# febrianrachmadi/dep-gan-im

Measured on AMD Instinct MI355X. Metric: 2D slices/sec (G+2D+GP train step), 256x256x1 fp32, higher is better.
Workload: dtype f32; 1 GPU; DEP-GAN-IM twoCritics canonical train step (critic-Y2 + critic-DEM + G update, WGAN-GP), batch 32 per GPU, 256x256x1; per_gpu_batch=32, global_batch=32, parallelism=dp1

## Files before the change

dep_gan_im_amd/csrc/common.h:

```cpp
#pragma once
#include <hip/hip_runtime.h>
#include <stdint.h>
#include <stddef.h>

typedef float f32x2 __attribute__((ext_vector_type(2)));
typedef float f32x4 __attribute__((ext_vector_type(4)));
typedef float f32x16 __attribute__((ext_vector_type(16)));

struct TView {
  float* p;
  long sB, sY, sX;
};

static inline TView make_view(float* p, int H, int W, int C) {
  TView v;
  v.p = p;
  v.sX = C;
  v.sY = (long)W * C;
  v.sB = (long)H * W * C;
  return v;
}
static inline TView make_view_slice(float* p, int H, int W, int Ctot, int c0) {
  TView v = make_view(p, H, W, Ctot);
  v.p = p + c0;
// ... 217 lines not shown
int dg_wino_epi_class(unsigned flags, int form);
void dg_set_epi_classes(int on);
int dg_get_epi_classes();
void dg_conv_igemm_name(const ConvPlan& pl, const ConvArgs& a, char* buf, size_t cap);
int dg_conv_direct(int KS, const ConvArgs& a, hipStream_t st);

size_t dg_wgrad_part_floats(int KS, int B, int H, int W, int Cin, int Cout);
int dg_wgrad(int KS, const WgradArgs& a, int* nchunks, hipStream_t st);
int dg_wgrad_finish(const float* part, int nchunks, int ntaps, int Cin, int Cout, const float* scale, float* out,
                    float* raw, int accumulate, int oi, const float* colpart, int colC, const float* colscale,
                    float* colout, float* colraw, hipStream_t st);
int dg_wgrad_finish_rows(const float* part, int nchunks, int ntaps, int Cin, int Cout, const float* scale, float* out,
                         float* raw, int accumulate, int oi, const float* colpart, int colrows, int colC,
                         const float* colscale, float* colout, float* colraw, hipStream_t st);
int dg_wgrad_reduce(const float* part, int nchunks, int ntaps, int Cin, int Cout, const float* scale, float* out,
                    float* raw, int accumulate, int oi, hipStream_t st);

bool dg_wgrad_bf16_supported(int KS, int Cin, int Cout);
size_t dg_wgrad_bf16_part_floats(int KS, int B, int H, int W, int Cin, int Cout);
int dg_wgrad_bf16(int KS, const WgradArgs& a, int* nchunks, hipStream_t st);

size_t dg_wgrad_small_part_floats(int KS, int B, int H, int W, int Cin, int Cout);
int dg_wgrad_small(int KS, const WgradArgs& a, int* nchunks, hipStream_t st);

int dg_wgrad_plan(int KS, int B, int H, int W, int Cin, int Cout, int out[4]);
int dg_wgrad_small_plan(int KS, int B, int H, int W, int Cin, int Cout, int out[4]);
int dg_wgrad_bf16_plan(int KS, int B, int H, int W, int Cin, int Cout, int out[4]);
```

dep_gan_im_amd/csrc/direct.hip:

```cpp
#include "common.h"
#include "epilogue.h"

template <int KS, int COG, int G>
__global__ __launch_bounds__(256) void conv_direct_kernel(const ConvArgs a) {
  constexpr int PAD = KS / 2;
  constexpr int TW = 16 + KS - 1;
  constexpr int PIXT = TW * TW;
  constexpr int NTAPS = KS * KS;
  constexpr int CT = COG * G;
  constexpr int CIK = 8;
  constexpr int PPP = 256 / G;
  constexpr int NPASS = G;

  extern __shared__ __attribute__((aligned(16))) float smem[];
  float* xs = smem;
  float* ws = smem + CIK * PIXT;

  const int tid = threadIdx.x;
  const int tilesX = (a.W + 15) >> 4, tilesY = (a.H + 15) >> 4;
  int t = blockIdx.x;
  const int tx0 = (t % tilesX) * 16;
  t /= tilesX;
  const int ty0 = (t % tilesY) * 16;
  const int b = t / tilesY;
// ... 349 lines not shown
      const int iy = ty0 + (pix >> 4), ix = tx0 + (pix & 15);
      float v = 0.f;
      if (iy < a.H && ix < a.W) v = a.dy.p[view_off(a.dy, b, iy, ix) + c];
      ds[pix * a.Cout + c] = v;
    }
    __syncthreads();
    for (int py = 0; py < 16; ++py)
#pragma unroll 4
      for (int px = 0; px < 16; ++px) {
        const int xo = py * TW + px;
        const int dof = (py * 16 + px) * a.Cout;
#pragma unroll
        for (int k = 0; k < NOUT; ++k) acc[k] = fmaf(xs[xoff[k] + xo], ds[dof + co_[k]], acc[k]);
      }
  }
  float* pout = a.part + (size_t)blockIdx.x * nout;
#pragma unroll
  for (int k = 0; k < NOUT; ++k) {
    const int o = tid + k * 256;
    if (o < nout) pout[o] = acc[k];
  }
}

template <int KS>
__global__ __launch_bounds__(256) void wgrad_edge_kernel(const WgradArgs a) {
  constexpr int PAD = KS / 2;
  constexpr int TW = 16 + KS - 1;
  constexpr int PIXT = TW * TW;
  constexpr int NTAPS = KS * KS;
  extern __shared__ __attribute__((aligned(16))) float smem[];
  const int xsz = (a.Cin * PIXT + 3) & ~3;
  float* xs = smem;
  float* ds = smem + xsz;
  const int tid = threadIdx.x, lane = tid & 63, wv = tid >> 6;
  const int i = lane & 15, kq = lane >> 4;
  const int M = NTAPS * a.Cin;
  const int MT = (M + 15) >> 4, NTl = a.Cout >> 4;
  int aoff[2];
  bool aval[2];
#pragma unroll
  for (int mt = 0; mt < 2; ++mt) {
    const int m = mt * 16 + i;
    aval[mt] = m < M;
    const int mm = aval[mt] ? m : 0;
    const int tap = mm / a.Cin, ci = mm - tap * a.Cin;
    aoff[mt] = ci * PIXT + (tap / KS) * TW + (tap % KS);
  }
  f32x4 acc[2][2];
#pragma unroll
  for (int mt = 0; mt < 2; ++mt)
#pragma unroll
    for (int nt = 0; nt < 2; ++nt) acc[mt][nt] = (f32x4){0.f, 0.f, 0.f, 0.f};
  const int tilesX = (a.W + 15) >> 4, tilesY = (a.H + 15) >> 4;
  const int t0 = blockIdx.x * a.tilesPerChunk, t1 = min(t0 + a.tilesPerChunk, a.nTiles);
  const int C4 = a.Cout >> 2;
  for (int tile = t0; tile < t1; ++tile) {
    int t = tile;
    const int tx0 = (t % tilesX) * 16;
    t /= tilesX;
    const int ty0 = (t % tilesY) * 16;
    const int b = t / tilesY;
    __syncthreads();
    for (int q = tid; q < PIXT * a.Cin; q += 256) {
      const int pix = q / a.Cin, c = q - pix * a.Cin;
      const int ly = pix / TW, lx = pix - ly * TW;
      const int iy = ty0 + ly - PAD, ix = tx0 + lx - PAD;
      float v = 0.f;
      if (iy >= 0 && iy < a.H && ix >= 0 && ix < a.W) v = a.x.p[view_off(a.x, b, iy, ix) + c];
      xs[c * PIXT + pix] = v;
    }
    for (int q = tid; q < 256 * C4; q += 256) {
      const int pix = q / C4, c = (q - pix * C4) * 4;
      const int iy = ty0 + (pix >> 4), ix = tx0 + (pix & 15);
      f32x4 v = {0.f, 0.f, 0.f, 0.f};
      if (iy < a.H && ix < a.W) v = *reinterpret_cast<const f32x4*>(a.dy.p + view_off(a.dy, b, iy, ix) + c);
      *reinterpret_cast<f32x4*>(ds + pix * a.Cout + c) = v;
    }
    __syncthreads();
#pragma unroll 4
    for (int kk = 0; kk < 16; ++kk) {
      const int kl = kk * 4 + kq;
      const int py = 4 * wv + (kl >> 4), px = kl & 15;
      const int po = py * TW + px;
      float av[2], bv[2];
#pragma unroll
      for (int mt = 0; mt < 2; ++mt) av[mt] = aval[mt] ? xs[aoff[mt] + po] : 0.f;
#pragma unroll
      for (int nt = 0; nt < 2; ++nt) bv[nt] = (nt < NTl) ? ds[(py * 16 + px) * a.Cout + nt * 16 + i] : 0.f;
#pragma unroll
      for (int mt = 0; mt < 2; ++mt)
#pragma unroll
        for (int nt = 0; nt < 2; ++nt)
          if (mt < MT && nt < NTl) acc[mt][nt] = __builtin_amdgcn_mfma_f32_16x16x4f32(av[mt], bv[nt], acc[mt][nt], 0, 0, 0);
    }
  }
  __syncthreads();
  float* red = smem;
#pragma unroll
  for (int mt = 0; mt < 2; ++mt)
#pragma unroll
    for (int nt = 0; nt < 2; ++nt)
#pragma unroll
      for (int j = 0; j < 4; ++j) red[wv * 1024 + (mt * 16 + 4 * kq + j) * 32 + nt * 16 + i] = acc[mt][nt][j];
  __syncthreads();
  float* pout = a.part + (size_t)blockIdx.x * M * a.Cout;
  for (int e = tid; e < M * a.Cout; e += 256) {
    const int m = e / a.Cout, n = e - m * a.Cout;
    const int o = m * 32 + n;
    pout[e] = (red[o] + red[1024 + o]) + (red[2048 + o] + red[3072 + o]);
  }
}

static void small_chunking(int B, int H, int W, int* nTiles, int* tpc, int* nch) {
  *nTiles = B * cdiv(W, 16) * cdiv(H, 16);
  int want = *nTiles / 6;
  if (want < 1024) want = 1024;
  if (want > 8192) want = 8192;
  if (want > *nTiles) want = *nTiles;
  *tpc = cdiv(*nTiles, want);
  *nch = cdiv(*nTiles, *tpc);
}

size_t dg_wgrad_small_part_floats(int KS, int B, int H, int W, int Cin, int Cout) {
  int nTiles, tpc, nch;
  small_chunking(B, H, W, &nTiles, &tpc, &nch);
  const size_t slab = (size_t)KS * KS * Cin * Cout;
  return (size_t)nch * slab;
}

int dg_wgrad_small_plan(int KS, int B, int H, int W, int Cin, int Cout, int out[4]) {
  if (KS * KS * Cin * Cout > 1024 || Cout > 64) {
    dg_set_error("dg_wgrad_small: taps*Cin*Cout = %d too large", KS * KS * Cin * Cout);
    return DG_ERR_UNSUPPORTED;
  }
  if (KS != 3 && KS != 5) {
    dg_set_error("dg_wgrad_small: unsupported kernel size %d", KS);
    return DG_ERR_UNSUPPORTED;
  }
  small_chunking(B, H, W, &out[0], &out[1], &out[2]);
  out[3] = 1;
  return DG_OK;
}

int dg_wgrad_small(int KS, const WgradArgs& a_in, int* nchunks, hipStream_t st) {
  WgradArgs a = a_in;
  if (KS * KS * a.Cin * a.Cout > 1024 || a.Cout > 64) {
    dg_set_error("dg_wgrad_small: taps*Cin*Cout = %d too large", KS * KS * a.Cin * a.Cout);
    return DG_ERR_UNSUPPORTED;
  }
  int nTiles, tpc, nch;
  small_chunking(a.B, a.H, a.W, &nTiles, &tpc, &nch);
  a.nTiles = nTiles;
  a.tilesPerChunk = tpc;
  *nchunks = nch;
  const int TW = 16 + KS - 1;
  const bool edge = (KS * KS * a.Cin <= 32) && (a.Cout == 16 || a.Cout == 32) && (a.dy.sX % 4 == 0) &&
                    (a.dy.sY % 4 == 0) && (a.dy.sB % 4 == 0);
  if (edge) {
    size_t lds = (size_t)(((a.Cin * TW * TW + 3) & ~3) + 256 * a.Cout) * sizeof(float);
    if (lds < 4 * 1024 * sizeof(float)) lds = 4 * 1024 * sizeof(float);
    if (KS == 3)
      hipLaunchKernelGGL(wgrad_edge_kernel<3>, dim3(nch), dim3(256), lds, st, a);
    else if (KS == 5)
      hipLaunchKernelGGL(wgrad_edge_kernel<5>, dim3(nch), dim3(256), lds, st, a);
    else {
      dg_set_error("dg_wgrad_small: unsupported kernel size %d", KS);
      return DG_ERR_UNSUPPORTED;
    }
    HIPCHECK(hipGetLastError());
    return DG_OK;
  }
  const size_t lds = (size_t)(a.Cin * TW * TW + 256 * a.Cout) * sizeof(float);
  if (KS == 3)
    hipLaunchKernelGGL(wgrad_small_kernel<3>, dim3(nch), dim3(256), lds, st, a);
  else if (KS == 5)
    hipLaunchKernelGGL(wgrad_small_kernel<5>, dim3(nch), dim3(256), lds, st, a);
  else {
    dg_set_error("dg_wgrad_small: unsupported kernel size %d", KS);
    return DG_ERR_UNSUPPORTED;
  }
// ... 4 lines not shown
```

dep_gan_im_amd/csrc/model.hip:

```cpp
#include "model.h"
#include "train_ops.h"

#include <dlfcn.h>
#include <float.h>
#include <math.h>
#include <stdlib.h>
#include <stdarg.h>
#include <stdio.h>
#include <string.h>

static thread_local char g_err[1024] = "";
void dg_set_error(const char* fmt, ...) {
  va_list ap;
  va_start(ap, fmt);
  vsnprintf(g_err, sizeof(g_err), fmt, ap);
  va_end(ap);
}
const char* dg_get_error() { return g_err; }

void Net::add(const std::string& name, std::vector<int> shape, bool trainable) {
  PInfo pi;
  pi.name = name;
  pi.ndim = (int)shape.size();
  pi.size = 1;
// ... 198 lines not shown
  int nch = 0;
  const double fl = 2.0 * N * H * W * (double)Cin * Cout * KS * KS;
  char lb[56];
  snprintf(lb, sizeof(lb), "wgrad k%d b%d %dx%d %d->%d", KS, N, H, W, Cin, Cout);
  const bool mfma = Cin % 4 == 0 && Cout % 4 == 0 && Cin >= 8;
  if (ws.bf16 && mfma && dg_wgrad_bf16_supported(KS, Cin, Cout)) {
    if (dg_wgrad_bf16_part_floats(KS, N, H, W, Cin, Cout) > ws.partFloats) {
      dg_set_error("wgrad slab workspace too small");
      return DG_ERR_ARG;
    }
    if (cs) {
      a.colpart = scratch;
      a.colB = cs->B;
    }
    snprintf(lb, sizeof(lb), "wgrad(bf16) k%d b%d %dx%d %d->%d", KS, N, H, W, Cin, Cout);
    {
      ProfScope ps(c, 1, fl, lb);
      DGCHECK(dg_wgrad_bf16(KS, a, &nch, ws.st));
    }
    ProfScope ps(c, 2, 0.0, "slab reduce");
    return dg_wgrad_finish(ws.part, nch, KS * KS, Cin, Cout, scale, out, raw, accumulate, oi, cs ? scratch : nullptr,
                           Cout, cs ? cs->scale : nullptr, cs ? cs->out : nullptr, cs ? cs->raw : nullptr, ws.st);
  }
  if (cs && !mfma) {
    ProfScope ps(c, 2, 0.0, "colsum");
    DGCHECK(dg_colsum(dy, cs->B, H, W, Cout, cs->scale, cs->out, cs->raw, 0, scratch, cap, ws.st));
  }
  if (mfma) {
    if (dg_wgrad_part_floats(KS, N, H, W, Cin, Cout) > ws.partFloats) {
      dg_set_error("wgrad slab workspace too small");
      return DG_ERR_ARG;
    }
    if (cs) {
      a.colpart = scratch;
      a.colB = cs->B;
    }
    {
      ProfScope ps(c, 1, fl, lb);
      DGCHECK(dg_wgrad(KS, a, &nch, ws.st));
    }
    ProfScope ps(c, 2, 0.0, "slab reduce");
    return dg_wgrad_finish(ws.part, nch, KS * KS, Cin, Cout, scale, out, raw, accumulate, oi, cs ? scratch : nullptr,
                           Cout, cs ? cs->scale : nullptr, cs ? cs->out : nullptr, cs ? cs->raw : nullptr, ws.st);
  } else {
    if (dg_wgrad_small_part_floats(KS, N, H, W, Cin, Cout) > ws.partFloats) {
      dg_set_error("wgrad slab workspace too small");
      return DG_ERR_ARG;
    }
    ProfScope ps(c, 2, fl, lb);
    DGCHECK(dg_wgrad_small(KS, a, &nch, ws.st));
  }
  ProfScope ps(c, 2, 0.0, "slab reduce");
  return dg_wgrad_reduce(ws.part, nch, KS * KS, Cin, Cout, scale, out, raw, accumulate, oi, ws.st);
}
int wgrad_full(depgan_ctx* c, int KS, TView x, TView dy, int N, int H, int W, int Cin, int Cout,
               const float* scale, float* out, float* raw, int accumulate, int oi, const ColSum* cs) {
  const WgradWs ws = {c->part, c->partFloats, c->scratch, c->scratchFloats, c->cfg.bf16_mfma && c->wgrad_bf16, c->st, c};
  return wgrad_run(ws, KS, x, dy, N, H, W, Cin, Cout, scale, out, raw, accumulate, oi, cs);
}

static const char* kHeadSfx[NOISE_NHEADS] = {"add_m3", "mul_m3", "add_m2", "mul_m2", "add_m1", "mul_m1", "add",
                                             "mul",    "add_p3", "mul_p3", "add_p2", "mul_p2", "add_p1", "mul_p1"};
static const int kHeadMult[NOISE_NHEADS] = {3, 3, 2, 2, 1, 1, 4, 4, 3, 3, 2, 2, 1, 1};

struct TrunkEnt {
  GKind kind;
  const char* name;
  int ci, co;
  const char* aux;
};
static const TrunkEnt kTrunk[] = {
    {G_CONV, "gen_0", -1, 1, ""},        {G_FILM, "gen_noise_m1", 1, 1, "m1"}, {G_CONV, "gen_1", 1, 1, ""},
    {G_POOL, "skip1", 0, 0, ""},         {G_CONV, "gen_2", 1, 2, ""},          {G_FILM, "gen_noise_m2", 2, 2, "m2"},
// ... 1507 lines not shown
```

dep_gan_im_amd/csrc/op_entries.hip:

```cpp
#include "model.h"
#include "train_ops.h"

#include <math.h>
#include <stdlib.h>
#include <stdio.h>
#include <string.h>

int op_pack_jobs(PackJob* jobs, int n, hipStream_t st) {
  const unsigned nb = dg_pack_layout(jobs, n);
  DevTmp jd(st);
  DGCHECK(jd.alloc(n * sizeof(PackJob)));
  hipError_t e = hipMemcpyAsync(jd.p, jobs, n * sizeof(PackJob), hipMemcpyHostToDevice, st);
  if (e != hipSuccess) { dg_set_error("op_pack_jobs: upload failed: %s", hipGetErrorString(e)); return DG_ERR_HIP; }
  return dg_pack_weights_batch(jd.as<PackJob>(), n, nb, st);
}

extern "C" {

static int op_conv_run(ConvArgs a, const float* w_hwio, int Cin, int Cout, int KS, int path, int bwd, hipStream_t st) {
  const int ci = a.Cin, co = a.Cout;
  ConvPlan pl = (path == 3) ? dg_plan_conv_bf16(KS, ci, co)
                : (path == 4 || path == 5) ? dg_plan_conv_split(KS, ci, co, path == 5 ? 3 : 2)
                : (path == 6) ? dg_plan_conv_items(KS, ci, co, 1L << 30) : dg_plan_conv(KS, ci, co);
  if (path == 7) pl = dg_plan_conv_items(KS, ci, co, 1L << 30);
// ... 359 lines not shown
                              long dsX, const float* scale, float* dw, float* raw, int accumulate, int oi,
                              int colB, const float* colscale, float* colout, float* colraw, int B, int H, int W,
                              int Cin, int Cout, int KS, int bf16, void* stream) {
  if (op_view_bad_batched(x, xsB, xsY, xsX) || op_view_bad_batched(dy, dsB, dsY, dsX) || !dw || B < 1 || H < 1 || W < 1 || Cin < 1 || Cout < 1 ||
      (KS != 1 && KS != 3 && KS != 5)) {
    dg_set_error("op_conv2d_wgrad_ex: null or non-positive argument");
    return DG_ERR_ARG;
  }
  const bool cols = colout || colraw;
  if ((bf16 != 0 && bf16 != 1) || (cols ? (colB < 1 || colB > B) : (colB != 0 || colscale != nullptr))) {
    dg_set_error("op_conv2d_wgrad_ex: bf16 must be 0 or 1; column sums need colout or colraw and 1 <= colB <= B");
    return DG_ERR_ARG;
  }
  const bool mfma = Cin % 4 == 0 && Cout % 4 == 0 && Cin >= 8;
  if (bf16 && !(mfma && dg_wgrad_bf16_supported(KS, Cin, Cout))) {
    dg_set_error("op_conv2d_wgrad_ex: the bf16 weight-gradient kernel does not cover %d -> %d", Cin, Cout);
    return DG_ERR_UNSUPPORTED;
  }
  hipStream_t st = (hipStream_t)stream;
  WgradWs ws;
  memset(&ws, 0, sizeof(ws));
  ws.partFloats = bf16 ? dg_wgrad_bf16_part_floats(KS, B, H, W, Cin, Cout)
                  : mfma ? dg_wgrad_part_floats(KS, B, H, W, Cin, Cout) : dg_wgrad_small_part_floats(KS, B, H, W, Cin, Cout);
  ws.scratchFloats = mfma ? ws.partFloats / ((size_t)KS * KS * Cin) : (cols ? dg_colsum_scratch(colB, H, W, Cout) : 0);
  ws.bf16 = bf16 != 0;
  ws.st = st;
  DevTmp part(st), scratch(st);
  DGCHECK(op_alloc(&part, ws.partFloats, "op_conv2d_wgrad_ex"));
  DGCHECK(op_alloc(&scratch, ws.scratchFloats, "op_conv2d_wgrad_ex"));
  ws.part = part.as<float>();
  ws.scratch = scratch.as<float>();
  const ColSum cs = {colB, colscale, colout, colraw};
  return wgrad_run(ws, KS, op_view(x, xsB, xsY, xsX), op_view(dy, dsB, dsY, dsX), B, H, W, Cin, Cout, scale, dw, raw, accumulate,
                   oi, cols ? &cs : nullptr);
}

int depgan_debug_wgrad_plan(int kernel, int KS, int B, int H, int W, int Cin, int Cout, int out[4]) {
  if (!out || B < 1 || H < 1 || W < 1 || Cin < 1 || Cout < 1) {
    dg_set_error("debug_wgrad_plan: null or non-positive argument");
    return DG_ERR_ARG;
  }
  switch (kernel) {
    case 0: return dg_wgrad_plan(KS, B, H, W, Cin, Cout, out);
    case 1: return dg_wgrad_small_plan(KS, B, H, W, Cin, Cout, out);
    case 2: return dg_wgrad_bf16_plan(KS, B, H, W, Cin, Cout, out);
    case 3: return dg_wgrad_bf16s_plan(KS, B, H, W, Cin, Cout, out);
    case 4: return dg_deconv_wgrad_plan(B, H, W, Cin, Cout, out);
// ... 584 lines not shown
```

dep_gan_im_amd/csrc/wgrad.hip:

```cpp
#include <stdlib.h>

#include "common.h"

template <int MF>
struct MfmaW;
template <>
struct MfmaW<32> {
  typedef f32x16 acc_t;
  static constexpr int NREG = 16;
  static __device__ __forceinline__ acc_t run(float a, float b, acc_t c) {
    return __builtin_amdgcn_mfma_f32_32x32x2f32(a, b, c, 0, 0, 0);
  }
  static __device__ __forceinline__ int row(int j, int h) { return (j & 3) + 8 * (j >> 2) + 4 * h; }
};
template <>
struct MfmaW<16> {
  typedef f32x4 acc_t;
  static constexpr int NREG = 4;
  static __device__ __forceinline__ acc_t run(float a, float b, acc_t c) {
    return __builtin_amdgcn_mfma_f32_16x16x4f32(a, b, c, 0, 0, 0);
  }
  static __device__ __forceinline__ int row(int j, int h) { return 4 * h + j; }
};

template <int MF, int KS, int TPW, int TH>
struct WDmaCfg {
  static constexpr int TW = 16 + KS - 1, THH = TH + KS - 1, PIXT = THH * TW, V = MF / 4;
  static constexpr int XTOT = PIXT * V, DTOT = TH * 16 * V;
  static constexpr int NXP = (XTOT + 255) / 256, NDP = DTOT / 256;
  static constexpr int XBUF = NXP * 256 * 4, DBUF = DTOT * 4, BUF = XBUF + DBUF;
  static constexpr size_t LDS_TILES = (size_t)2 * BUF * sizeof(float);
  static constexpr bool TWO_PER_CU = (MF == 32 && KS == 3 && TH == 8) || (MF == 32 && KS == 5 && TH == 4);
  static constexpr int RT = TWO_PER_CU ? (KS == 3 ? 3 : 1) : TPW;
  static constexpr size_t LDS_RED = (size_t)RT * 4 * MF * MF * sizeof(float);
  static constexpr size_t LDS_BYTES = LDS_TILES > LDS_RED ? LDS_TILES : LDS_RED;
  static constexpr int WGS_PER_CU = TWO_PER_CU ? 2 : 1;
  static_assert(DTOT % 256 == 0, "dy tile must be whole wave-instructions");
};

template <int MF, int KS, int TPW, int TH>
__global__ __launch_bounds__(256, (WDmaCfg<MF, KS, TPW, TH>::WGS_PER_CU)) void wgrad_dma_kernel(const WgradArgs a) {
  typedef WDmaCfg<MF, KS, TPW, TH> C;
  constexpr int PAD = KS / 2, TW = C::TW, NTAPS = KS * KS, NGT = NTAPS / TPW;
  constexpr int KM = 64 / MF, PW = TH * 4, KSTEPS = PW / KM, V = C::V;
  constexpr int XTOT = C::XTOT, NXP = C::NXP, NDP = C::NDP, XBUF = C::XBUF, BUF = C::BUF;
  constexpr int NPIECE = NXP + NDP;
  constexpr int NREAD = TPW + 1;
  constexpr bool COUNTED = NREAD <= 15;
  static_assert(NTAPS % TPW == 0 && (TPW == NTAPS || TPW == KS), "tap grouping");
  static_assert(NPIECE <= 63, "vmcnt is a 6-bit counter");
  typedef typename MfmaW<MF>::acc_t acc_t;

  extern __shared__ __attribute__((aligned(16))) float smem[];

  const int tid = threadIdx.x, lane = tid & 63, wv = tid >> 6;
  const int r = lane % MF, h = lane / MF;
  const int nCoT = (a.Cout + MF - 1) / MF;
  int y, chunk;
  {
    const unsigned nY = gridDim.y, nX = gridDim.x;
    const unsigned id = blockIdx.x + blockIdx.y * nX;
    if ((nX & 7u) == 0 && nY > 1) {
      const unsigned x = id & 7u, sl = id >> 3;
      y = (int)(sl % nY);
      chunk = (int)(8u * (sl / nY) + x);
    } else {
      y = (int)blockIdx.y;
      chunk = (int)blockIdx.x;
    }
  }
  const int tg = y % NGT;
  y /= NGT;
  const int co0 = (y % nCoT) * MF;
  const int ci0 = (y / nCoT) * MF;
  const int tilesX = (a.W + 15) >> 4, tilesY = (a.H + TH - 1) / TH;
  const int t0 = chunk * a.tilesPerChunk;
  const int t1 = min(t0 + a.tilesPerChunk, a.nTiles);

  acc_t acc[TPW];
#pragma unroll
  for (int t = 0; t < TPW; ++t)
#pragma unroll
    for (int j = 0; j < MfmaW<MF>::NREG; ++j) acc[t][j] = 0.f;

  const float* const xorg = a.x.p + ci0 - PAD * ((long)a.x.sY + (long)a.x.sX);
  const float* const dorg = a.dy.p + co0;
  constexpr int SENT = (int)0x80000000;
  int xvo[NXP], xyx[NXP];
#pragma unroll
  for (int i = 0; i < NXP; ++i) {
    const int q = tid + i * 256;
    const int pix = q / V, part = q & (V - 1);
    const int ly = pix / TW, lx = pix - ly * TW;
    const bool ok = q < XTOT && (ci0 + part * 4) < a.Cin;
    xvo[i] = ok ? 4 * (ly * (int)a.x.sY + lx * (int)a.x.sX + part * 4) : SENT;
    xyx[i] = (ly << 8) | lx;
  }
  constexpr int DROWS = 256 / V / 16;
  const int dly = (tid / V) >> 4, dlx = (tid / V) & 15;
  const int dvo = ((co0 + (tid & (V - 1)) * 4) < a.Cout)
                      ? 4 * (dly * (int)a.dy.sY + dlx * (int)a.dy.sX + (tid & (V - 1)) * 4)
                      : SENT;
  const int dstep = 4 * DROWS * (int)a.dy.sY;
  const int wbase = __builtin_amdgcn_readfirstlane(wv * 256);

  const bool do_cs = a.colpart != nullptr && ci0 == 0 && tg == 0;
  float cs0 = 0.f, cs1 = 0.f;
  int bq[2] = {0, 0};
  int ntx, nty, nb;
  {
    int t = t0;
    ntx = t % tilesX;
    t /= tilesX;
    nty = t % tilesY;
    nb = t / tilesY;
  }

  const int fragB = ((wv * (TH / 4)) * 16 + h) * MF + r;
  const int fragX = ((wv * (TH / 4) + (TPW == NTAPS ? 0 : tg)) * TW + h) * MF + r;

  for (int tile = t0 - 1; tile < t1; ++tile) {
    const int buf = (tile - t0) & 1;
    __builtin_amdgcn_s_barrier();
    if (tile + 1 < t1) {
      const int tx0 = ntx * 16, ty0 = nty * TH;
      const int xso = 4 * (nb * (int)a.x.sB + ty0 * (int)a.x.sY + tx0 * (int)a.x.sX);
      const int dso = 4 * (nb * (int)a.dy.sB + ty0 * (int)a.dy.sY + tx0 * (int)a.dy.sX);
      const bool interior = ty0 >= PAD && ty0 + TH + PAD <= a.H && tx0 >= PAD && tx0 + 16 + PAD <= a.W;
      float* xs = smem + (buf ^ 1) * BUF + wbase;
      float* ds = xs + XBUF;
      bq[buf ^ 1] = nb;
      auto mkrsrc = [](const float* p) {
        const unsigned long long u = (unsigned long long)p;
        const unsigned lo = __builtin_amdgcn_readfirstlane((unsigned)u);
        const unsigned hi = __builtin_amdgcn_readfirstlane((unsigned)(u >> 32));
        return __builtin_amdgcn_make_buffer_rsrc((void*)(((unsigned long long)hi << 32) | lo), 0, 0x7FFFFFFF,
                                                 0x00020000);
      };
      const __amdgpu_buffer_rsrc_t rx = mkrsrc(xorg), rd = mkrsrc(dorg);
      if (interior) {
#pragma unroll
        for (int i = 0; i < NXP; ++i) {
          const int vo = xvo[i];
          __builtin_amdgcn_raw_ptr_buffer_load_lds(rx, (__attribute__((address_space(3))) void*)(xs + i * 1024), 16,
                                                   vo, xso, 0, 0);
        }
#pragma unroll
        for (int i = 0; i < NDP; ++i)
          __builtin_amdgcn_raw_ptr_buffer_load_lds(rd, (__attribute__((address_space(3))) void*)(ds + i * 1024), 16,
                                                   dvo, dso + i * dstep, 0, 0);
      } else {
#pragma unroll
        for (int i = 0; i < NXP; ++i) {
          const int iy = ty0 + (xyx[i] >> 8) - PAD, ix = tx0 + (xyx[i] & 255) - PAD;
          const int vo = (iy >= 0 && iy < a.H && ix >= 0 && ix < a.W) ? xvo[i] : SENT;
          __builtin_amdgcn_raw_ptr_buffer_load_lds(rx, (__attribute__((address_space(3))) void*)(xs + i * 1024), 16,
                                                   vo, xso, 0, 0);
        }
#pragma unroll
        for (int i = 0; i < NDP; ++i) {
          const int vo = ((ty0 + dly + i * DROWS) < a.H && (tx0 + dlx) < a.W) ? dvo : SENT;
          __builtin_amdgcn_raw_ptr_buffer_load_lds(rd, (__attribute__((address_space(3))) void*)(ds + i * 1024), 16,
                                                   vo, dso + i * dstep, 0, 0);
        }
      }
      if (++ntx == tilesX) {
        ntx = 0;
        if (++nty == tilesY) {
          nty = 0;
          ++nb;
        }
      }
      asm volatile("s_waitcnt vmcnt(%0)" ::"n"(NPIECE) : "memory");
    } else {
      asm volatile("s_waitcnt vmcnt(0)" ::: "memory");
    }
    __builtin_amdgcn_s_barrier();
    if (tile < t0) continue;
    const float csmul = (do_cs && bq[buf] < a.colB) ? 1.0f : 0.0f;
    if (COUNTED) {
      const unsigned bbase =
          (unsigned)(size_t)(__attribute__((address_space(3))) float*)(smem + buf * BUF + XBUF + fragB);
      const unsigned xbase = (unsigned)(size_t)(__attribute__((address_space(3))) float*)(smem + buf * BUF + fragX);
      const unsigned xb[4] = {xbase, xbase + 64u, xbase + 128u, xbase + 192u};
      static_assert(KSTEPS % 2 == 0 && (16 / KM) % 2 == 0, "k-steps are paired inside a pixel row");
// ... 40 lines not shown
        const int pyo = kk / SPR, pxo = (kk % SPR) * KM;
        bv = bbase[(pyo * 16 + pxo) * MF];
#pragma unroll
        for (int tl = 0; tl < TPW; ++tl) {
          const int ty = (TPW == NTAPS) ? (tl / KS) : 0;
          const int tx = (TPW == NTAPS) ? (tl % KS) : tl;
          av[tl] = xbase[((pyo + ty) * TW + pxo + tx) * MF];
        }
      };
      load_frag(0, afr[0], bfr[0]);
#pragma unroll
      for (int kk = 0; kk < KSTEPS; ++kk) {
        if (kk + 1 < KSTEPS) load_frag(kk + 1, afr[(kk + 1) & 1], bfr[(kk + 1) & 1]);
        __builtin_amdgcn_sched_barrier(0);
#pragma unroll
        for (int tl = 0; tl < TPW; ++tl) acc[tl] = MfmaW<MF>::run(afr[kk & 1][tl], bfr[kk & 1], acc[tl]);
        cs0 = fmaf(bfr[kk & 1], csmul, cs0);
        __builtin_amdgcn_sched_barrier(0);
      }
    }
  }

  constexpr int RT = C::RT;
  float* red = smem;
  const size_t slab = (size_t)NTAPS * a.Cin * a.Cout;
  float* pout = a.part + (size_t)chunk * slab;
#pragma unroll
  for (int t0 = 0; t0 < TPW; t0 += RT) {
    __syncthreads();
#pragma unroll
    for (int tl = 0; tl < RT; ++tl)
#pragma unroll
      for (int j = 0; j < MfmaW<MF>::NREG; ++j)
        red[(tl * 4 + wv) * MF * MF + MfmaW<MF>::row(j, h) * MF + r] = acc[t0 + tl][j];
    __syncthreads();
    for (int q = tid; q < RT * MF * MF; q += 256) {
      const int tl = q / (MF * MF), e = q % (MF * MF);
      const float* rt = red + tl * 4 * MF * MF;
      const float sum = (rt[e] + rt[MF * MF + e]) + (rt[2 * MF * MF + e] + rt[3 * MF * MF + e]);
      const int tap = tg * TPW + t0 + tl;
      const int ci = ci0 + e / MF, co = co0 + e % MF;
      if (ci < a.Cin && co < a.Cout) pout[((size_t)tap * a.Cin + ci) * a.Cout + co] = sum;
    }
  }
  if (do_cs) {
    __syncthreads();
    red[tid] = cs0 + cs1;
    __syncthreads();
    if (tid < MF) {
      float s = 0.f;
#pragma unroll
      for (int w = 0; w < 4; ++w)
#pragma unroll
        for (int hh = 0; hh < 64 / MF; ++hh) s += red[w * 64 + hh * MF + tid];
      if (co0 + tid < a.Cout) a.colpart[(size_t)chunk * a.Cout + co0 + tid] = s;
    }
  }
}

struct WVar {
  int MF, KS, TPW, TH;
  size_t lds;
};

static bool wgrad_th8() {
  static int on = -1;
  if (on < 0) {
    const char* e = getenv("DEPGAN_WGRAD_TH8");
    on = (e && atoi(e) == 0) ? 0 : 1;
  }
  return on != 0;
}

static void pick_variant(int KS, int Cin, int Cout, WVar* v) {
  v->KS = KS;
  v->MF = (Cin % 32 == 0 && Cout % 32 == 0) ? 32 : 16;
  v->TH = 16;
  v->TPW = KS * KS;
  if (KS == 5 && v->MF == 32) {
    v->TPW = 5;
    v->TH = wgrad_th8() ? 4 : 8;
  }
  if (KS == 3 && v->MF == 32 && wgrad_th8()) v->TH = 8;
  v->lds = 0;
  if (KS == 3 && v->MF == 32) v->lds = v->TH == 8 ? WDmaCfg<32, 3, 9, 8>::LDS_BYTES : WDmaCfg<32, 3, 9, 16>::LDS_BYTES;
  if (KS == 3 && v->MF == 16) v->lds = WDmaCfg<16, 3, 9, 16>::LDS_BYTES;
  if (KS == 5 && v->MF == 32) v->lds = v->TH == 4 ? WDmaCfg<32, 5, 5, 4>::LDS_BYTES : WDmaCfg<32, 5, 5, 8>::LDS_BYTES;
  if (KS == 5 && v->MF == 16) v->lds = WDmaCfg<16, 5, 25, 16>::LDS_BYTES;
  if (KS == 1 && v->MF == 32) v->lds = WDmaCfg<32, 1, 1, 16>::LDS_BYTES;
  if (KS == 1 && v->MF == 16) v->lds = WDmaCfg<16, 1, 1, 16>::LDS_BYTES;
}

// ... 14 lines not shown
  WVar v;
  pick_variant(KS, Cin, Cout, &v);
  int nTiles, tpc, nch, gy;
  chunking(v, B, H, W, Cin, Cout, &nTiles, &tpc, &nch, &gy);
  const size_t slab = (size_t)KS * KS * Cin * Cout;
  return (size_t)nch * slab;
}

int dg_wgrad_plan(int KS, int B, int H, int W, int Cin, int Cout, int out[4]) {
  if ((Cin % 4) || (Cout % 4)) {
    dg_set_error("dg_wgrad: channels and strides must be multiples of 4 floats (Cin=%d Cout=%d)", Cin, Cout);
    return DG_ERR_ARG;
  }
  if (KS != 1 && KS != 3 && KS != 5) {
    dg_set_error("dg_wgrad: unsupported kernel size %d", KS);
    return DG_ERR_UNSUPPORTED;
  }
  WVar v;
  pick_variant(KS, Cin, Cout, &v);
  chunking(v, B, H, W, Cin, Cout, &out[0], &out[1], &out[2], &out[3]);
  return DG_OK;
}

template <int MF, int KS, int TPW, int TH>
static int launch_wgrad_dma(WgradArgs a, int nchunks, int gridY, hipStream_t st) {
  constexpr size_t lds = WDmaCfg<MF, KS, TPW, TH>::LDS_BYTES;
  static_assert(lds <= 160 * 1024, "two tile buffers must fit the CU's LDS");
  static DgOncePerDevice once;
  if (once.need()) {
    HIPCHECK(hipFuncSetAttribute(reinterpret_cast<const void*>(&wgrad_dma_kernel<MF, KS, TPW, TH>),
                                 hipFuncAttributeMaxDynamicSharedMemorySize, (int)lds));
  }
  hipLaunchKernelGGL((wgrad_dma_kernel<MF, KS, TPW, TH>), dim3(nchunks, gridY), dim3(256), lds, st, a);
  HIPCHECK(hipGetLastError());
  return DG_OK;
}

int dg_wgrad(int KS, const WgradArgs& a_in, int* nchunks_out, hipStream_t st) {
  WgradArgs a = a_in;
  if ((a.Cin % 4) || (a.Cout % 4) || (a.x.sX % 4) || (a.x.sY % 4) || (a.x.sB % 4) || (a.dy.sX % 4) ||
      (a.dy.sY % 4) || (a.dy.sB % 4) || (((uintptr_t)a.x.p) & 15) || (((uintptr_t)a.dy.p) & 15)) {
    dg_set_error("dg_wgrad: channels and strides must be multiples of 4 floats (Cin=%d Cout=%d)", a.Cin, a.Cout);
    return DG_ERR_ARG;
  }
  const long long lim = 0x7FFFFFFFll - (1ll << 20);
  if ((long long)a.B * a.x.sB * 4 + ((long long)a.x.sY + a.x.sX) * 4 * KS >= lim || (long long)a.B * a.dy.sB * 4 >= lim) {
    dg_set_error("dg_wgrad: operand spans 2 GiB or more (B=%d, batch strides %ld / %ld floats)", a.B, (long)a.x.sB,
                 (long)a.dy.sB);
    return DG_ERR_UNSUPPORTED;
  }
  WVar v;
  pick_variant(KS, a.Cin, a.Cout, &v);
  int nTiles, tpc, nch, gy;
  chunking(v, a.B, a.H, a.W, a.Cin, a.Cout, &nTiles, &tpc, &nch, &gy);
  a.nTiles = nTiles;
  a.tilesPerChunk = tpc;
  *nchunks_out = nch;
  if (KS == 3 && v.MF == 32 && v.TH == 8) return launch_wgrad_dma<32, 3, 9, 8>(a, nch, gy, st);
  if (KS == 3 && v.MF == 32) return launch_wgrad_dma<32, 3, 9, 16>(a, nch, gy, st);
  if (KS == 3 && v.MF == 16) return launch_wgrad_dma<16, 3, 9, 16>(a, nch, gy, st);
  if (KS == 5 && v.MF == 32 && v.TH == 4) return launch_wgrad_dma<32, 5, 5, 4>(a, nch, gy, st);
  if (KS == 5 && v.MF == 32) return launch_wgrad_dma<32, 5, 5, 8>(a, nch, gy, st);
  if (KS == 5 && v.MF == 16) return launch_wgrad_dma<16, 5, 25, 16>(a, nch, gy, st);
  if (KS == 1 && v.MF == 32) return launch_wgrad_dma<32, 1, 1, 16>(a, nch, gy, st);
  if (KS == 1 && v.MF == 16) return launch_wgrad_dma<16, 1, 1, 16>(a, nch, gy, st);
  dg_set_error("dg_wgrad: unsupported kernel size %d", KS);
  return DG_ERR_UNSUPPORTED;
}

struct ColFin {
  const float* part;
  const float* scale;
  float *out, *raw;
  int nb, C;
};
template <int SL>
__global__ __launch_bounds__(64 * SL) void slab_reduce_kernel(const float* __restrict__ in, int nin, int ntaps, int Cin,
                                                              int Cout, const float* __restrict__ scale,
                                                              float* __restrict__ out, float* __restrict__ raw,
                                                              int accumulate, int oi, unsigned nbr, ColFin cf) {
  __shared__ float sh[64 * SL];
  if (blockIdx.x >= nbr) {
    const int c = (int)(blockIdx.x - nbr);
    float s = 0.f;
    for (int b = threadIdx.x; b < cf.nb; b += 64 * SL) s += cf.part[(size_t)b * cf.C + c];
// ... 78 lines not shown
```

Measured before the change: 712.6 slices/s.

## Fuse bias column sums into edge wgrad kernel; run 8-wave MF16 k5 wgrad

The small edge weight-gradient kernel now also accumulates per-channel column sums of dy (the bias gradient) while it already has dy in registers. This removes the separate colsum kernel and its extra read of dy, and the partial sums are reduced in the existing finish-rows pass. Separately, the MF16 5x5 DMA wgrad kernel is generalised to a configurable wave count and now defaults to 8 waves (512 threads) per workgroup, which gives more latency hiding and less work per wave at the cost of a larger cross-wave reduction. Both paths can be turned off through environment variables.

```diff
diff --git a/dep_gan_im_amd/csrc/common.h b/dep_gan_im_amd/csrc/common.h
--- a/dep_gan_im_amd/csrc/common.h
+++ b/dep_gan_im_amd/csrc/common.h
@@ -263,6 +263,7 @@
 
 size_t dg_wgrad_small_part_floats(int KS, int B, int H, int W, int Cin, int Cout);
 int dg_wgrad_small(int KS, const WgradArgs& a, int* nchunks, hipStream_t st);
+bool dg_wgrad_edge_colsum(int KS, const WgradArgs& a);
 
 int dg_wgrad_plan(int KS, int B, int H, int W, int Cin, int Cout, int out[4]);
 int dg_wgrad_small_plan(int KS, int B, int H, int W, int Cin, int Cout, int out[4]);
diff --git a/dep_gan_im_amd/csrc/direct.hip b/dep_gan_im_amd/csrc/direct.hip
--- a/dep_gan_im_amd/csrc/direct.hip
+++ b/dep_gan_im_amd/csrc/direct.hip
@@ -1,3 +1,5 @@
+#include <stdlib.h>
+
 #include "common.h"
 #include "epilogue.h"
 
@@ -395,8 +397,8 @@
   }
 }
 
-template <int KS>
-__global__ __launch_bounds__(256) void wgrad_edge_kernel(const WgradArgs a) {
+template <int KS, bool CS>
+static __device__ __forceinline__ void wgrad_edge_body(const WgradArgs& a) {
   constexpr int PAD = KS / 2;
   constexpr int TW = 16 + KS - 1;
   constexpr int PIXT = TW * TW;
@@ -427,12 +429,14 @@
   const int tilesX = (a.W + 15) >> 4, tilesY = (a.H + 15) >> 4;
   const int t0 = blockIdx.x * a.tilesPerChunk, t1 = min(t0 + a.tilesPerChunk, a.nTiles);
   const int C4 = a.Cout >> 2;
+  float cs[2] = {0.f, 0.f};
   for (int tile = t0; tile < t1; ++tile) {
     int t = tile;
     const int tx0 = (t % tilesX) * 16;
     t /= tilesX;
     const int ty0 = (t % tilesY) * 16;
     const int b = t / tilesY;
+    const float csmul = (CS && b < a.colB) ? 1.0f : 0.0f;
     __syncthreads();
     for (int q = tid; q < PIXT * a.Cin; q += 256) {
       const int pix = q / a.Cin, c = q - pix * a.Cin;
@@ -460,6 +464,10 @@
       for (int mt = 0; mt < 2; ++mt) av[mt] = aval[mt] ? xs[aoff[mt] + po] : 0.f;
 #pragma unroll
       for (int nt = 0; nt < 2; ++nt) bv[nt] = (nt < NTl) ? ds[(py * 16 + px) * a.Cout + nt * 16 + i] : 0.f;
+      if (CS) {
+#pragma unroll
+        for (int nt = 0; nt < 2; ++nt) cs[nt] = fmaf(bv[nt], csmul, cs[nt]);
+      }
 #pragma unroll
       for (int mt = 0; mt < 2; ++mt)
 #pragma unroll
@@ -482,6 +490,26 @@
     const int o = m * 32 + n;
     pout[e] = (red[o] + red[1024 + o]) + (red[2048 + o] + red[3072 + o]);
   }
+  if (CS) {
+    __syncthreads();
+    red[tid * 2] = cs[0];
+    red[tid * 2 + 1] = cs[1];
+    __syncthreads();
+    if (tid < a.Cout) {
+      const int nt = tid >> 4, ii = tid & 15;
+      float s = 0.f;
+#pragma unroll
+      for (int w = 0; w < 4; ++w)
+#pragma unroll
+        for (int q = 0; q < 4; ++q) s += red[(w * 64 + q * 16 + ii) * 2 + nt];
+      a.colpart[(size_t)blockIdx.x * a.Cout + tid] = s;
+    }
+  }
+}
+template <int KS>
+__global__ __launch_bounds__(256) void wgrad_edge_kernel(const WgradArgs a) {
+  if (a.colpart) wgrad_edge_body<KS, true>(a);
+  else wgrad_edge_body<KS, false>(a);
 }
 
 static void small_chunking(int B, int H, int W, int* nTiles, int* tpc, int* nch) {
@@ -515,6 +543,19 @@
   return DG_OK;
 }
 
+static bool wgrad_small_is_edge(int KS, const WgradArgs& a) {
+  return (KS == 3 || KS == 5) && (KS * KS * a.Cin <= 32) && (a.Cout == 16 || a.Cout == 32) && (a.dy.sX % 4 == 0) &&
+         (a.dy.sY % 4 == 0) && (a.dy.sB % 4 == 0);
+}
+bool dg_wgrad_edge_colsum(int KS, const WgradArgs& a) {
+  static int on = -1;
+  if (on < 0) {
+    const char* e = getenv("DEPGAN_WGRAD_EDGE_COLSUM");
+    on = (e && atoi(e) == 0) ? 0 : 1;
+  }
+  return on != 0 && KS * KS * a.Cin * a.Cout <= 1024 && wgrad_small_is_edge(KS, a);
+}
+
 int dg_wgrad_small(int KS, const WgradArgs& a_in, int* nchunks, hipStream_t st) {
   WgradArgs a = a_in;
   if (KS * KS * a.Cin * a.Cout > 1024 || a.Cout > 64) {
@@ -527,8 +568,11 @@
   a.tilesPerChunk = tpc;
   *nchunks = nch;
   const int TW = 16 + KS - 1;
-  const bool edge = (KS * KS * a.Cin <= 32) && (a.Cout == 16 || a.Cout == 32) && (a.dy.sX % 4 == 0) &&
-                    (a.dy.sY % 4 == 0) && (a.dy.sB % 4 == 0);
+  const bool edge = wgrad_small_is_edge(KS, a);
+  if (a.colpart && !edge) {
+    dg_set_error("dg_wgrad_small: column sums ride in wgrad_edge_kernel only (k%d %d -> %d)", KS, a.Cin, a.Cout);
+    return DG_ERR_UNSUPPORTED;
+  }
   if (edge) {
     size_t lds = (size_t)(((a.Cin * TW * TW + 3) & ~3) + 256 * a.Cout) * sizeof(float);
     if (lds < 4 * 1024 * sizeof(float)) lds = 4 * 1024 * sizeof(float);
diff --git a/dep_gan_im_amd/csrc/model.hip b/dep_gan_im_amd/csrc/model.hip
--- a/dep_gan_im_amd/csrc/model.hip
+++ b/dep_gan_im_amd/csrc/model.hip
@@ -244,7 +244,8 @@
     return dg_wgrad_finish(ws.part, nch, KS * KS, Cin, Cout, scale, out, raw, accumulate, oi, cs ? scratch : nullptr,
                            Cout, cs ? cs->scale : nullptr, cs ? cs->out : nullptr, cs ? cs->raw : nullptr, ws.st);
   }
-  if (cs && !mfma) {
+  const bool edge_cs = cs && !mfma && dg_wgrad_edge_colsum(KS, a);
+  if (cs && !mfma && !edge_cs) {
     ProfScope ps(c, 2, 0.0, "colsum");
     DGCHECK(dg_colsum(dy, cs->B, H, W, Cout, cs->scale, cs->out, cs->raw, 0, scratch, cap, ws.st));
   }
@@ -269,8 +270,24 @@
       dg_set_error("wgrad slab workspace too small");
       return DG_ERR_ARG;
     }
-    ProfScope ps(c, 2, fl, lb);
-    DGCHECK(dg_wgrad_small(KS, a, &nch, ws.st));
+    if (edge_cs) {
+      const size_t rows = dg_wgrad_small_part_floats(KS, N, H, W, Cin, Cout) / ((size_t)KS * KS * Cin * Cout);
+      if (rows * Cout > cap) {
+        dg_set_error("wgrad column-sum workspace too small (%zu floats, %zu needed)", cap, rows * Cout);
+        return DG_ERR_ARG;
+      }
+      a.colpart = scratch;
+      a.colB = cs->B;
+    }
+    {
+      ProfScope ps(c, 2, fl, lb);
+      DGCHECK(dg_wgrad_small(KS, a, &nch, ws.st));
+    }
+    if (edge_cs) {
+      ProfScope ps(c, 2, 0.0, "slab reduce");
+      return dg_wgrad_finish_rows(ws.part, nch, KS * KS, Cin, Cout, scale, out, raw, accumulate, oi, scratch, nch, Cout,
+                                  cs->scale, cs->out, cs->raw, ws.st);
+    }
   }
   ProfScope ps(c, 2, 0.0, "slab reduce");
   return dg_wgrad_reduce(ws.part, nch, KS * KS, Cin, Cout, scale, out, raw, accumulate, oi, ws.st);
diff --git a/dep_gan_im_amd/csrc/op_entries.hip b/dep_gan_im_amd/csrc/op_entries.hip
--- a/dep_gan_im_amd/csrc/op_entries.hip
+++ b/dep_gan_im_amd/csrc/op_entries.hip
@@ -405,7 +405,9 @@
   memset(&ws, 0, sizeof(ws));
   ws.partFloats = bf16 ? dg_wgrad_bf16_part_floats(KS, B, H, W, Cin, Cout)
                   : mfma ? dg_wgrad_part_floats(KS, B, H, W, Cin, Cout) : dg_wgrad_small_part_floats(KS, B, H, W, Cin, Cout);
-  ws.scratchFloats = mfma ? ws.partFloats / ((size_t)KS * KS * Cin) : (cols ? dg_colsum_scratch(colB, H, W, Cout) : 0);
+  const size_t rowFloats = ws.partFloats / ((size_t)KS * KS * Cin);
+  ws.scratchFloats = mfma ? rowFloats : (cols ? dg_colsum_scratch(colB, H, W, Cout) : 0);
+  if (!mfma && cols && ws.scratchFloats < rowFloats) ws.scratchFloats = rowFloats;
   ws.bf16 = bf16 != 0;
   ws.st = st;
   DevTmp part(st), scratch(st);
diff --git a/dep_gan_im_amd/csrc/wgrad.hip b/dep_gan_im_amd/csrc/wgrad.hip
--- a/dep_gan_im_amd/csrc/wgrad.hip
+++ b/dep_gan_im_amd/csrc/wgrad.hip
@@ -23,26 +23,33 @@
   static __device__ __forceinline__ int row(int j, int h) { return 4 * h + j; }
 };
 
-template <int MF, int KS, int TPW, int TH>
-struct WDmaCfg {
+template <int MF, int KS, int TPW, int TH, int NW_>
+struct WDmaCfgN {
+  static constexpr int NW = NW_, NT = 64 * NW;
   static constexpr int TW = 16 + KS - 1, THH = TH + KS - 1, PIXT = THH * TW, V = MF / 4;
   static constexpr int XTOT = PIXT * V, DTOT = TH * 16 * V;
-  static constexpr int NXP = (XTOT + 255) / 256, NDP = DTOT / 256;
-  static constexpr int XBUF = NXP * 256 * 4, DBUF = DTOT * 4, BUF = XBUF + DBUF;
+  static constexpr int NXP = (XTOT + NT - 1) / NT, NDP = DTOT / NT;
+  static constexpr int XBUF = NXP * NT * 4, DBUF = DTOT * 4, BUF = XBUF + DBUF;
   static constexpr size_t LDS_TILES = (size_t)2 * BUF * sizeof(float);
   static constexpr bool TWO_PER_CU = (MF == 32 && KS == 3 && TH == 8) || (MF == 32 && KS == 5 && TH == 4);
-  static constexpr int RT = TWO_PER_CU ? (KS == 3 ? 3 : 1) : TPW;
-  static constexpr size_t LDS_RED = (size_t)RT * 4 * MF * MF * sizeof(float);
+  static constexpr int RT = TWO_PER_CU ? (KS == 3 ? 3 : 1) : (NW == 8 ? 5 : TPW);
+  static constexpr size_t LDS_RED = (size_t)RT * NW * MF * MF * sizeof(float);
   static constexpr size_t LDS_BYTES = LDS_TILES > LDS_RED ? LDS_TILES : LDS_RED;
   static constexpr int WGS_PER_CU = TWO_PER_CU ? 2 : 1;
-  static_assert(DTOT % 256 == 0, "dy tile must be whole wave-instructions");
+  static constexpr int WAVES_PER_SIMD = WGS_PER_CU * NW / 4;
+  static_assert(NW == 4 || NW == 8, "the final sum is written for 4 or 8 waves");
+  static_assert(DTOT % NT == 0, "dy tile must be whole wave-instructions");
+  static_assert(TH % NW == 0 && TPW % RT == 0, "rows per wave, taps per reduction round");
 };
-
 template <int MF, int KS, int TPW, int TH>
-__global__ __launch_bounds__(256, (WDmaCfg<MF, KS, TPW, TH>::WGS_PER_CU)) void wgrad_dma_kernel(const WgradArgs a) {
-  typedef WDmaCfg<MF, KS, TPW, TH> C;
+struct WDmaCfg : WDmaCfgN<MF, KS, TPW, TH, (MF == 16 && KS == 5 && TPW == 25 && TH == 16) ? 8 : 4> {};
+
+template <int MF, int KS, int TPW, int TH, int NW>
+static __device__ __forceinline__ void wgrad_dma_body(const WgradArgs& a) {
+  typedef WDmaCfgN<MF, KS, TPW, TH, NW> C;
+  constexpr int NT = C::NT;
   constexpr int PAD = KS / 2, TW = C::TW, NTAPS = KS * KS, NGT = NTAPS / TPW;
-  constexpr int KM = 64 / MF, PW = TH * 4, KSTEPS = PW / KM, V = C::V;
+  constexpr int KM = 64 / MF, PW = TH * 16 / NW, KSTEPS = PW / KM, V = C::V;
   constexpr int XTOT = C::XTOT, NXP = C::NXP, NDP = C::NDP, XBUF = C::XBUF, BUF = C::BUF;
   constexpr int NPIECE = NXP + NDP;
   constexpr int NREAD = TPW + 1;
@@ -89,14 +96,14 @@
   int xvo[NXP], xyx[NXP];
 #pragma unroll
   for (int i = 0; i < NXP; ++i) {
-    const int q = tid + i * 256;
+    const int q = tid + i * NT;
     const int pix = q / V, part = q & (V - 1);
     const int ly = pix / TW, lx = pix - ly * TW;
     const bool ok = q < XTOT && (ci0 + part * 4) < a.Cin;
     xvo[i] = ok ? 4 * (ly * (int)a.x.sY + lx * (int)a.x.sX + part * 4) : SENT;
     xyx[i] = (ly << 8) | lx;
   }
-  constexpr int DROWS = 256 / V / 16;
+  constexpr int DROWS = NT / V / 16;
   const int dly = (tid / V) >> 4, dlx = (tid / V) & 15;
   const int dvo = ((co0 + (tid & (V - 1)) * 4) < a.Cout)
                       ? 4 * (dly * (int)a.dy.sY + dlx * (int)a.dy.sX + (tid & (V - 1)) * 4)
@@ -116,8 +123,8 @@
     nb = t / tilesY;
   }
 
-  const int fragB = ((wv * (TH / 4)) * 16 + h) * MF + r;
-  const int fragX = ((wv * (TH / 4) + (TPW == NTAPS ? 0 : tg)) * TW + h) * MF + r;
+  const int fragB = ((wv * (TH / NW)) * 16 + h) * MF + r;
+  const int fragX = ((wv * (TH / NW) + (TPW == NTAPS ? 0 : tg)) * TW + h) * MF + r;
 
   for (int tile = t0 - 1; tile < t1; ++tile) {
     const int buf = (tile - t0) & 1;
@@ -142,25 +149,25 @@
 #pragma unroll
         for (int i = 0; i < NXP; ++i) {
           const int vo = xvo[i];
-          __builtin_amdgcn_raw_ptr_buffer_load_lds(rx, (__attribute__((address_space(3))) void*)(xs + i * 1024), 16,
+          __builtin_amdgcn_raw_ptr_buffer_load_lds(rx, (__attribute__((address_space(3))) void*)(xs + i * (NT * 4)), 16,
                                                    vo, xso, 0, 0);
         }
 #pragma unroll
         for (int i = 0; i < NDP; ++i)
-          __builtin_amdgcn_raw_ptr_buffer_load_lds(rd, (__attribute__((address_space(3))) void*)(ds + i * 1024), 16,
+          __builtin_amdgcn_raw_ptr_buffer_load_lds(rd, (__attribute__((address_space(3))) void*)(ds + i * (NT * 4)), 16,
                                                    dvo, dso + i * dstep, 0, 0);
       } else {
 #pragma unroll
         for (int i = 0; i < NXP; ++i) {
           const int iy = ty0 + (xyx[i] >> 8) - PAD, ix = tx0 + (xyx[i] & 255) - PAD;
           const int vo = (iy >= 0 && iy < a.H && ix >= 0 && ix < a.W) ? xvo[i] : SENT;
-          __builtin_amdgcn_raw_ptr_buffer_load_lds(rx, (__attribute__((address_space(3))) void*)(xs + i * 1024), 16,
+          __builtin_amdgcn_raw_ptr_buffer_load_lds(rx, (__attribute__((address_space(3))) void*)(xs + i * (NT * 4)), 16,
                                                    vo, xso, 0, 0);
         }
 #pragma unroll
         for (int i = 0; i < NDP; ++i) {
           const int vo = ((ty0 + dly + i * DROWS) < a.H && (tx0 + dlx) < a.W) ? dvo : SENT;
-          __builtin_amdgcn_raw_ptr_buffer_load_lds(rd, (__attribute__((address_space(3))) void*)(ds + i * 1024), 16,
+          __builtin_amdgcn_raw_ptr_buffer_load_lds(rd, (__attribute__((address_space(3))) void*)(ds + i * (NT * 4)), 16,
                                                    vo, dso + i * dstep, 0, 0);
         }
       }
@@ -247,6 +254,7 @@
   }
 
   constexpr int RT = C::RT;
+  constexpr int MM = MF * MF;
   float* red = smem;
   const size_t slab = (size_t)NTAPS * a.Cin * a.Cout;
   float* pout = a.part + (size_t)chunk * slab;
@@ -257,12 +265,13 @@
     for (int tl = 0; tl < RT; ++tl)
 #pragma unroll
       for (int j = 0; j < MfmaW<MF>::NREG; ++j)
-        red[(tl * 4 + wv) * MF * MF + MfmaW<MF>::row(j, h) * MF + r] = acc[t0 + tl][j];
+        red[(tl * NW + wv) * MM + MfmaW<MF>::row(j, h) * MF + r] = acc[t0 + tl][j];
     __syncthreads();
-    for (int q = tid; q < RT * MF * MF; q += 256) {
-      const int tl = q / (MF * MF), e = q % (MF * MF);
-      const float* rt = red + tl * 4 * MF * MF;
-      const float sum = (rt[e] + rt[MF * MF + e]) + (rt[2 * MF * MF + e] + rt[3 * MF * MF + e]);
+    for (int q = tid; q < RT * MM; q += NT) {
+      const int tl = q / MM, e = q % MM;
+      const float* rt = red + tl * NW * MM;
+      float sum = (rt[e] + rt[MM + e]) + (rt[2 * MM + e] + rt[3 * MM + e]);
+      if (NW == 8) sum += (rt[4 * MM + e] + rt[5 * MM + e]) + (rt[6 * MM + e] + rt[7 * MM + e]);
       const int tap = tg * TPW + t0 + tl;
       const int ci = ci0 + e / MF, co = co0 + e % MF;
       if (ci < a.Cin && co < a.Cout) pout[((size_t)tap * a.Cin + ci) * a.Cout + co] = sum;
@@ -275,12 +284,22 @@
     if (tid < MF) {
       float s = 0.f;
 #pragma unroll
-      for (int w = 0; w < 4; ++w)
+      for (int w = 0; w < NW; ++w)
 #pragma unroll
         for (int hh = 0; hh < 64 / MF; ++hh) s += red[w * 64 + hh * MF + tid];
       if (co0 + tid < a.Cout) a.colpart[(size_t)chunk * a.Cout + co0 + tid] = s;
     }
   }
+}
+
+template <int MF, int KS, int TPW, int TH>
+__global__ __launch_bounds__((WDmaCfg<MF, KS, TPW, TH>::NT), (WDmaCfg<MF, KS, TPW, TH>::WAVES_PER_SIMD)) void
+wgrad_dma_kernel(const WgradArgs a) {
+  wgrad_dma_body<MF, KS, TPW, TH, WDmaCfg<MF, KS, TPW, TH>::NW>(a);
+}
+template <int MF, int KS, int TPW, int TH>
+__global__ __launch_bounds__(256, 1) void wgrad_dma_kernel_w4(const WgradArgs a) {
+  wgrad_dma_body<MF, KS, TPW, TH, 4>(a);
 }
 
 struct WVar {
@@ -293,6 +312,15 @@
   if (on < 0) {
     const char* e = getenv("DEPGAN_WGRAD_TH8");
     on = (e && atoi(e) == 0) ? 0 : 1;
+  }
+  return on != 0;
+}
+
+static bool wgrad_mf16_waves8() {
+  static int on = -1;
+  if (on < 0) {
+    const char* e = getenv("DEPGAN_WGRAD_MF16_WAVES");
+    on = (e && atoi(e) == 4) ? 0 : 1;
   }
   return on != 0;
 }
@@ -353,18 +381,27 @@
   return DG_OK;
 }
 
+template <void (*KERNEL)(const WgradArgs), int THREADS, size_t LDS>
+static int launch_wdma(WgradArgs a, int nchunks, int gridY, hipStream_t st) {
+  static_assert(LDS <= 160 * 1024, "two tile buffers must fit the CU's LDS");
+  static DgOncePerDevice once;
+  if (once.need()) {
+    HIPCHECK(hipFuncSetAttribute(reinterpret_cast<const void*>(KERNEL), hipFuncAttributeMaxDynamicSharedMemorySize,
+                                 (int)LDS));
+  }
+  hipLaunchKernelGGL(KERNEL, dim3(nchunks, gridY), dim3(THREADS), LDS, st, a);
+  HIPCHECK(hipGetLastError());
+  return DG_OK;
+}
 template <int MF, int KS, int TPW, int TH>
 static int launch_wgrad_dma(WgradArgs a, int nchunks, int gridY, hipStream_t st) {
-  constexpr size_t lds = WDmaCfg<MF, KS, TPW, TH>::LDS_BYTES;
-  static_assert(lds <= 160 * 1024, "two tile buffers must fit the CU's LDS");
-  static DgOncePerDevice once;
-  if (once.need()) {
-    HIPCHECK(hipFuncSetAttribute(reinterpret_cast<const void*>(&wgrad_dma_kernel<MF, KS, TPW, TH>),
-                                 hipFuncAttributeMaxDynamicSharedMemorySize, (int)lds));
-  }
-  hipLaunchKernelGGL((wgrad_dma_kernel<MF, KS, TPW, TH>), dim3(nchunks, gridY), dim3(256), lds, st, a);
-  HIPCHECK(hipGetLastError());
-  return DG_OK;
+  typedef WDmaCfg<MF, KS, TPW, TH> C;
+  return launch_wdma<&wgrad_dma_kernel<MF, KS, TPW, TH>, C::NT, C::LDS_BYTES>(a, nchunks, gridY, st);
+}
+template <int MF, int KS, int TPW, int TH>
+static int launch_wgrad_dma_w4(WgradArgs a, int nchunks, int gridY, hipStream_t st) {
+  typedef WDmaCfgN<MF, KS, TPW, TH, 4> C;
+  return launch_wdma<&wgrad_dma_kernel_w4<MF, KS, TPW, TH>, C::NT, C::LDS_BYTES>(a, nchunks, gridY, st);
 }
 
 int dg_wgrad(int KS, const WgradArgs& a_in, int* nchunks_out, hipStream_t st) {
@@ -392,6 +429,7 @@
   if (KS == 3 && v.MF == 16) return launch_wgrad_dma<16, 3, 9, 16>(a, nch, gy, st);
   if (KS == 5 && v.MF == 32 && v.TH == 4) return launch_wgrad_dma<32, 5, 5, 4>(a, nch, gy, st);
   if (KS == 5 && v.MF == 32) return launch_wgrad_dma<32, 5, 5, 8>(a, nch, gy, st);
+  if (KS == 5 && v.MF == 16 && !wgrad_mf16_waves8()) return launch_wgrad_dma_w4<16, 5, 25, 16>(a, nch, gy, st);
   if (KS == 5 && v.MF == 16) return launch_wgrad_dma<16, 5, 25, 16>(a, nch, gy, st);
   if (KS == 1 && v.MF == 32) return launch_wgrad_dma<32, 1, 1, 16>(a, nch, gy, st);
   if (KS == 1 && v.MF == 16) return launch_wgrad_dma<16, 1, 1, 16>(a, nch, gy, st);
```

New measurement: 718.0 slices/s, median of 6. No clear change (+0.8%).
